# teasgen/speech_separation

Measured on AMD Instinct MI355X. Metric: mixtures/sec (2-spk, 4 s @ 8 kHz) DPTN-AV forward, higher is better.
Workload: dtype f32; 1 GPU; configs[2]: DPTN-AV (dptn_wav_av) forward, precomputed lip embeddings, batch=16 per GPU, T=32000, random-init weights (numpy seed 0); batch_per_gpu=16, samples=32000, parallelism=dp1 (batch shards, no data-path collective)

## Files before the change

speech_separation_amd/csrc/dptnav.hip:

```cpp
#include <hip/hip_runtime.h>

#include <cmath>
#include <cstdarg>
#include <cstdio>
#include <cstring>
#include <string>
#include <vector>

#include "../../include/dptnav.h"
#include "attention.h"
#include "attn_long_train.h"
#include "attn_block.h"
#include "attn_block64.h"
#include "common.h"
#include "gemm_ws.h"
#include "headtail.h"
#include "lstm.h"
#include "lstm16.h"
#include "fcln.h"
#include "dgrad_t.h"
#include "dgrad_r.h"
#include "gemm_t.h"
#include "sisnr.h"
#include "train_tail.h"
// ... 4 lines not shown
namespace {

thread_local std::string g_create_error;

struct PathWeights {
  const float *in_w, *in_b, *out_w, *out_b, *ln1_w, *ln1_b;
  const float *w_ih[2], *w_hh[2], *b_ih[2], *b_hh[2];
  const float *ffn_w, *ffn_b, *ln2_w, *ln2_b;
  int ndir;
};

constexpr int QUEUE_SLOTS = 1024;

struct Plan {
  int64_t L, S, M;
  size_t queue, vid, E, X0, X1, qkv, att, y1, pre, hc, stamps, wfold, wpack, wih, whh4, winp, wmask, total;
  size_t qkv_n, att_n, y1_n, hc_n;
};

struct Run {
  float* ws;
  Plan pl;
  hipStream_t st;
  int slot;
  hipEvent_t lstm_wait = nullptr;
  hipEvent_t lstm_record = nullptr;
  int half = 0;
  bool packed_whh4 = false;
  bool packed_inw = false;
  bool packed_wih = false;
  bool fuse128 = false;
  int batch_total = 0;
  bool packed = false;
  unsigned* take_queue(int n) {
    unsigned* q = reinterpret_cast<unsigned*>(ws + pl.queue) + slot;
    slot += n;
    return q;
  }
};

}

enum ProfCat { CAT_VIDEO = 0, CAT_ENCODER, CAT_QKV, CAT_ATTN, CAT_OUTPROJ, CAT_LSTM_PRE, CAT_LSTM, CAT_FFN,
// ... 4 lines not shown

struct ProfRec {
  int cat;
  hipEvent_t a, b;
};

struct dptnav_ctx {
  dptnav_config cfg;
  bool prof_on = false;
  bool opt_lstm_stamps = false;
  bool opt_overlap = true;
  bool opt_serialize = false;
  bool opt_lstm16 = true;
  int opt_fuse_pre128 = 1;
  int opt_lstm_sched = 1;
  bool fuse128_for(int B) const { return opt_fuse_pre128 == 2 || (opt_fuse_pre128 == 1 && B >= 12); }
  int opt_fcln = 1;
  bool opt_fuse_pre = true;
  bool opt_pack_whh = true;
  bool opt_pack_wih = true;
  bool opt_deterministic = false;
  int opt_lstm4 = 1;
  bool opt_split_bf16 = false;
  bool opt_fuse_attn = true;
  bool opt_gemm_t = true;
  bool opt_dgrad_r = true;
  bool opt_dgrad_t = true;
  bool opt_attn_v2 = true;
  int opt_attn_persist = 1;
  bool opt_fold_tail = true;
// ... 275 lines not shown
  p->X1 = take((size_t)p->M * N);
  p->qkv_n = (size_t)p->M * 3 * N;
  p->qkv = take(p->qkv_n);
  p->att_n = (size_t)p->M * N;
  p->att = take(std::max(p->att_n, (size_t)2 * B * p->L * 8));
  p->y1_n = (size_t)p->M * N;
  p->y1 = take(p->y1_n);
  p->pre = take((size_t)2 * pre_tiles * 512 * 32);
  p->hc_n = (size_t)p->M * 2 * H;
  p->hc = take(p->hc_n + (size_t)p->S * g.chunk_size * 2 * H);
  p->stamps = take((size_t)2 * 2 * (nst_a > nst_e ? nst_a : nst_e) * 4 * 4 * 2);
  p->wfold = take((size_t)8 * 2 * N + 8);
  p->wpack = take(g.arch == 0 && N == 128 ? (size_t)2 * g.num_blocks * ATTN_PACK_FLOATS : 0);
  p->wih = take((size_t)2 * g.num_blocks * 2 * 4 * H * N);
  p->whh4 = take((size_t)2 * g.num_blocks * 2 * 4 * H * H);
  p->winp = take(g.arch == 0 && N == 128 ? (size_t)2 * g.num_blocks * 3 * N * N : 0);
  p->wmask = take(g.mask_tail ? (size_t)2 * N * N + 2 * N : 0);
  p->total = o;
  return DPTNAV_OK;
}

#define LAUNCH_CHECK(c, what)                                                                  \
  do {                                                                                          \
    if ((c)->opt_debug_sync) fprintf(stderr, "[dptnav] launched %s\n", what);                   \
    hipError_t e_ = hipGetLastError();                                                          \
    if (e_ != hipSuccess) return (c)->fail(DPTNAV_ERR_HIP, "%s: %s", what, hipGetErrorString(e_)); \
  } while (0)

template <class Kern>
int set_lds(dptnav_ctx* c, Kern kern, size_t bytes, const char* what) {
// ... 419 lines not shown
    } else if (use16) {
      EpiLstmPre16 ep{pre, {w.b_ih[0], w.b_ih[1]}, {w.b_hh[0], w.b_hh[1]}, geom, nst16};
      rc = launch_gemm<N, 4, 1, 4>(c, run, CAT_LSTM_PRE, "lstm-pre gemm", wih0, nt4, w.ndir, al, ep, wih1, ldw_ih);
    } else if (split) {
      EpiLstmPre ep{pre, {w.b_ih[0], w.b_ih[1]}, {w.b_hh[0], w.b_hh[1]}, geom};
      rc = launch_gemm<N, 4, 1, 4, false, true>(c, run, CAT_LSTM_PRE, "lstm-pre gemm (split)", w.w_ih[0], nt4, w.ndir, al, ep, w.w_ih[1]);
    } else {
      EpiLstmPre ep{pre, {w.b_ih[0], w.b_ih[1]}, {w.b_hh[0], w.b_hh[1]}, geom};
      rc = launch_gemm<N, 4, 1, 4>(c, run, CAT_LSTM_PRE, "lstm-pre gemm", wih0, nt4, w.ndir, al, ep, wih1, ldw_ih);
    }
    if (rc) return rc;
  }
  if (run.lstm_wait && hipStreamWaitEvent(st, run.lstm_wait, 0) != hipSuccess)
    return c->fail(DPTNAV_ERR_HIP, "lstm stagger wait");
  if (usex) {
    ProfScope ps(c, CAT_LSTM, st);
    const int rc = lstm16x_launch(N, dptn, nst16, w.ndir, st, lstm_in, N, w.w_ih, w.b_ih, w.b_hh, w.w_hh, hc, w.ndir * LSTM_H,
                                  M, geom, c->opt_lstm_sched);
    if (rc != 0) return c->fail(DPTNAV_ERR_HIP, "lstm16x: %s", hipGetErrorString((hipError_t)rc));
  } else if (use16 && split) {
    ProfScope ps(c, CAT_LSTM, st);
    const int rc = lstm16s_launch(c->cfg.arch == 0, nst16, w.ndir, st, pre, w.w_hh[0], w.w_hh[1], hc, w.ndir * LSTM_H, (int)M, geom);
    if (rc != 0) return c->fail(DPTNAV_ERR_HIP, "lstm16s: %s", hipGetErrorString((hipError_t)rc));
  } else if (use4) {
    const float *whh0 = w.w_hh[0], *whh1 = w.w_hh[1];
    if (c->opt_pack_whh && 2 * (int)c->pw.size() <= LSTM4_PACK_MAX) {
      float* base = ws + pl.whh4;
      if (!run.packed_whh4) {
        const float* src[LSTM4_PACK_MAX];
        for (size_t i = 0; i < c->pw.size(); ++i) {
          src[2 * i] = c->pw[i].w_hh[0];
          src[2 * i + 1] = c->pw[i].ndir == 2 ? c->pw[i].w_hh[1] : nullptr;
        }
// ... 1060 lines not shown
  if (ws == nullptr || ((uintptr_t)ws & 255) != 0)
    return c->fail(DPTNAV_ERR_WORKSPACE, "workspace must be non-null and 256-byte aligned");
  if (ws_bytes < pl->total * sizeof(float))
    return c->fail(DPTNAV_ERR_WORKSPACE, "workspace too small: %zu < %zu bytes", ws_bytes, pl->total * sizeof(float));
  return DPTNAV_OK;
}

int begin_run(dptnav_ctx* c, Run* run, float* ws, const Plan& pl, hipStream_t st) {
  run->ws = ws;
  run->pl = pl;
  run->st = st;
  run->slot = 0;
  run->packed = false;
  run->packed_wih = false;
  run->packed_whh4 = false;
  hipError_t e = hipMemsetAsync(ws + pl.queue, 0, QUEUE_SLOTS * sizeof(unsigned), st);
  if (e != hipSuccess) return c->fail(DPTNAV_ERR_HIP, "ticket counter reset: %s", hipGetErrorString(e));
  return DPTNAV_OK;
}

int join_after(dptnav_ctx* c, hipStream_t st, bool forked, int rc_body, int nstreams = 2) {
  if (!forked) return rc_body;
  const std::string body_err = c->err;
  bool ok = true;
  for (int s = 0; s < nstreams; ++s)
    ok &= hipEventRecord(c->ev_join[s], c->streams[s]) == hipSuccess && hipStreamWaitEvent(st, c->ev_join[s], 0) == hipSuccess;
  if (rc_body) {
    c->err = body_err;
    return rc_body;
  }
// ... 713 lines not shown

int dptnav_set_option(dptnav_handle h, const char* key, int value) {
  if (!h || !key) return DPTNAV_ERR_INVALID;
  const std::string k(key);
  if (k == "lstm_stamps") h->opt_lstm_stamps = value != 0;
  else if (k == "dropout_ppm" && value >= 0 && value < 1000000) h->opt_dropout_ppm = value;
  else if (k == "dropout_seed") h->opt_dropout_seed = (unsigned)value;
  else if (k == "overlap") h->opt_overlap = value != 0;
  else if (k == "serialize") h->opt_serialize = value != 0;
  else if (k == "deterministic") h->opt_deterministic = value != 0;
  else if (k == "pack_wih") h->opt_pack_wih = value != 0;
  else if (k == "fuse_pre") h->opt_fuse_pre = value != 0;
  else if (k == "fcln" && value >= 0 && value <= 2) h->opt_fcln = value;
  else if (k == "fuse_pre128" && value >= 0 && value <= 2) h->opt_fuse_pre128 = value;
  else if (k == "lstm_sched" && value >= 0 && value <= 1) h->opt_lstm_sched = value;
  else if (k == "pack_whh") h->opt_pack_whh = value != 0;
  else if (k == "lstm16") h->opt_lstm16 = value != 0;
  else if (k == "lstm4") {
    if (value < 0 || value > 2) return h->fail(DPTNAV_ERR_INVALID, "lstm4: 0, 1 or 2");
    h->opt_lstm4 = (int)value;
  }
  else if (k == "fuse_attn") h->opt_fuse_attn = value != 0;
  else if (k == "attn_v2") h->opt_attn_v2 = value != 0;
  else if (k == "attn_persist" && value >= 0) h->opt_attn_persist = value;
  else if (k == "dgrad_t") h->opt_dgrad_t = value != 0;
  else if (k == "dgrad_r") h->opt_dgrad_r = value != 0;
  else if (k == "gemm_t") h->opt_gemm_t = value != 0;
  else if (k == "fuse_ffn") h->opt_fuse_ffn = value != 0;
  else if (k == "wgrad2") h->opt_wgrad2 = value != 0;
  else if (k == "ln_tape") h->opt_ln_tape = value != 0;
// ... 78 lines not shown
```

speech_separation_amd/csrc/lstm16.h:

```cpp
#pragma once
#include "common.h"

constexpr int L16_H = 128;
constexpr int L16_LDH = L16_H + 8;
constexpr int L16_HS_FLOATS = 2 * 16 * L16_LDH;
constexpr int L16_PRE_FLOATS = 4 * 8 * 256;
constexpr size_t L16_LDS_BYTES = sizeof(float) * (L16_HS_FLOATS + L16_PRE_FLOATS);
constexpr int L16_TILE_FLOATS = 4 * L16_H * 16;

DEV constexpr float l16_gate_scale(int gate) { return gate == 2 ? -2.8853900817779268f : -1.4426950408889634f; }

DEV int64_t pre16_tile_offset(int d, int st16, int t, int nst16, int len) {
  return (((int64_t)d * nst16 + st16) * len + t) * (int64_t)L16_TILE_FLOATS;
}

constexpr int L16_VARIANT_TRAIN = 7;
int lstm16_launch(int variant, bool relu, int nst16, int ndir, void* stream, const float* pre, const float* whh_f,
                  const float* whh_b, float* hc, int ldh, int dump_row, const SeqGeom& g, unsigned long long* stamps,
                  float* tape_gates = nullptr, float* tape_c = nullptr);

int lstm16s_launch(bool relu, int nst16, int ndir, void* stream, const float* pre, const float* whh_f, const float* whh_b,
                   float* hc, int ldh, int dump_row, const SeqGeom& g);
int lstm32s_launch(bool relu, int nst, int ndir, void* stream, const float* pre, const float* whh_f, const float* whh_b, float* hc,
                   int ldh, int dump_row, const SeqGeom& g);

int lstm4_launch(bool relu, int nst4, int nst16, int ndir, void* stream, const float* pre, const float* whh_f,
                 const float* whh_b, float* hc, int ldh, int dump_row, const SeqGeom& g, bool packed = false);
constexpr int LSTM4_PACK_MAX = 24;
int lstm4_pack_launch(void* stream, const float* const* src, int n, float* dst);

int lstm16x_launch(int nin, bool relu, int nst16, int ndir, void* stream, const float* x, int ldx, const float* const* wih,
                   const float* const* bih, const float* const* bhh, const float* const* whh, float* hc, int ldh,
                   int64_t dump_row, const SeqGeom& g, int sched = 1);
```

speech_separation_amd/csrc/lstm16x.hip:

```cpp
#include <hip/hip_runtime.h>

#include "lstm16.h"
#include "vmem_asm.h"

namespace {

template <int NIN>
struct X16 {
  static constexpr int MK = NIN / 16;
  static constexpr int LDX = NIN + 8;
  static constexpr int WL_FLOATS = 4 * MK * 8 * 256;
  static constexpr int XS_FLOATS = 2 * 16 * LDX;
  static constexpr int NXL = (16 * NIN / 4) / 256;
  static constexpr size_t LDS_BYTES = sizeof(float) * (WL_FLOATS + L16_HS_FLOATS + XS_FLOATS);
  static_assert((16 * NIN / 4) % 256 == 0 && NIN % 16 == 0, "input tile / threads");
  static_assert(LDS_BYTES <= 160 * 1024, "W_ih must fit the LDS beside the h and x tiles");
};

template <int NIN, bool RELU>
__global__ __launch_bounds__(256) void lstm16x_kernel(const float* __restrict__ x, int ldx, const float* __restrict__ wih_f,
                                                       const float* __restrict__ wih_b, const float* __restrict__ bih_f,
                                                       const float* __restrict__ bih_b, const float* __restrict__ bhh_f,
                                                       const float* __restrict__ bhh_b, const float* __restrict__ whh_f,
                                                       const float* __restrict__ whh_b, float* __restrict__ hc, int ldh,
                                                       int64_t dump_row, SeqGeom g) {
  using Sh = X16<NIN>;
  constexpr int MK = Sh::MK, LDX = Sh::LDX, NXL = Sh::NXL;
  extern __shared__ __attribute__((aligned(16))) float smem[];
  float* Wl = smem;
  float* Hs = smem + Sh::WL_FLOATS;
  float* Xs = Hs + L16_HS_FLOATS;
  const int tid = threadIdx.x;
  const int w = __builtin_amdgcn_readfirstlane(tid >> 6);
  const int lane = tid & 63, i16 = lane & 15, ks = lane >> 4;
  const int st = blockIdx.x, d = blockIdx.y;
  const float* whh = d ? whh_b : whh_f;
  const float* wih = d ? wih_b : wih_f;
  const float* bih = d ? bih_b : bih_f;
  const float* bhh = d ? bhh_b : bhh_f;

  float wf[8][32];
  float bsc[8];
  float* wl_wave = Wl + w * (MK * 8 * 256) + lane * 4;
#pragma unroll
  for (int b = 0; b < 8; ++b) {
    const int row = (b >> 1) * L16_H + 32 * w + 16 * (b & 1) + i16;
    const float gs = l16_gate_scale(b >> 1);
    const float* wrow = whh + (int64_t)row * L16_H + 4 * ks;
#pragma unroll
    for (int m = 0; m < 8; ++m) {
      const float4 v = *reinterpret_cast<const float4*>(wrow + 16 * m);
      wf[b][4 * m + 0] = v.x * gs;
      wf[b][4 * m + 1] = v.y * gs;
      wf[b][4 * m + 2] = v.z * gs;
      wf[b][4 * m + 3] = v.w * gs;
    }
    bsc[b] = (bih[row] + bhh[row]) * gs;
    const float* irow = wih + (int64_t)row * NIN + 4 * ks;
#pragma unroll
    for (int m = 0; m < MK; ++m) {
      const float4 v = *reinterpret_cast<const float4*>(irow + 16 * m);
      *reinterpret_cast<float4*>(wl_wave + (m * 8 + b) * 256) = make_float4(v.x * gs, v.y * gs, v.z * gs, v.w * gs);
    }
  }
#pragma unroll
  for (int b = 0; b < 8; ++b)
#pragma unroll
    for (int i = 0; i < 32; ++i) asm volatile("" : "+a"(wf[b][i]));

  const int t0 = d ? g.len - 1 : 0, tdir = d ? -1 : 1;
  const int tstride = seq_token_stride(g);
  const int srow = 4 * w + (lane >> 5), scol = 4 * (lane & 31);
  char* hp[2];
  const int64_t hstep = (int64_t)tdir * tstride * ldh * 4;
#pragma unroll
  for (int j = 0; j < 2; ++j) {
    const int q = st * 16 + srow + 2 * j;
    const int64_t tokb = q < g.nseq ? seq_token_base(g, q) : dump_row;
    hp[j] = reinterpret_cast<char*>(hc) + ((tokb + (int64_t)t0 * tstride) * ldh + d * L16_H + scol) * 4;
  }
  const char* xp[NXL];
  int xoff[NXL];
  const int64_t xstep = (int64_t)tdir * tstride * ldx * 4;
// ... 10 lines not shown
    const int64_t adv = (int64_t)(s < g.len ? s : g.len - 1) * xstep;
#pragma unroll
    for (int i = 0; i < NXL; ++i) xr[i] = *reinterpret_cast<const float4*>(xp[i] + adv);
  };
  auto stage_x = [&](int buf) {
#pragma unroll
    for (int i = 0; i < NXL; ++i) *reinterpret_cast<float4*>(Xs + buf * 16 * LDX + xoff[i]) = xr[i];
  };
  load_x(0);
  stage_x(0);
  load_x(1);
  stage_x(1);
  load_x(2);
  for (int i = tid; i < 16 * L16_LDH; i += 256) Hs[i] = 0.f;
  f32x4v cst[2] = {(f32x4v){0.f, 0.f, 0.f, 0.f}, (f32x4v){0.f, 0.f, 0.f, 0.f}};
  __syncthreads();

  f32x4v acc[8];
  auto input_part = [&](int buf) {
#pragma unroll
    for (int b = 0; b < 8; ++b) acc[b] = (f32x4v){bsc[b], bsc[b], bsc[b], bsc[b]};
    const float* xrow = Xs + buf * 16 * LDX + i16 * LDX + 4 * ks;
    float4 xa[MK];
#pragma unroll
    for (int m = 0; m < MK; ++m) xa[m] = *reinterpret_cast<const float4*>(xrow + 16 * m);
    float4 wcur[8];
#pragma unroll
    for (int b = 0; b < 8; ++b) wcur[b] = *reinterpret_cast<const float4*>(wl_wave + b * 256);
#pragma unroll
    for (int m = 0; m < MK; ++m) {
// ... 78 lines not shown
      if (hf == 0) cell_half(0);
    }
    cell_half(1);
    if (step + 1 < g.len) input_part((step + 1) & 1);
    __syncthreads();
  }
  {
    const float* hfin = Hs + (g.len & 1) * 16 * L16_LDH;
#pragma unroll
    for (int j = 0; j < 2; ++j) {
      float4 v = *reinterpret_cast<const float4*>(hfin + (srow + 2 * j) * L16_LDH + scol);
      if (RELU) v = make_float4(relu1(v.x), relu1(v.y), relu1(v.z), relu1(v.w));
      *reinterpret_cast<float4*>(hp[j]) = v;
    }
  }
}

constexpr int X128_RES = 33;
constexpr int X128_WL_FLOATS = 4 * (64 - X128_RES) * 256;
constexpr int X128_XS_FLOATS = 16 * 128;
constexpr size_t X128_LDS_BYTES = sizeof(float) * (X128_WL_FLOATS + L16_HS_FLOATS + 2 * X128_XS_FLOATS);
static_assert(X128_LDS_BYTES <= 160 * 1024, "LDS budget");

DEV LstmCell2 lstm_cell2_fc(f32x2 ai, f32x2 af, f32x2 ag, f32x2 ao, f32x2 c_prev) {
  LstmCell2 r;
  r.i = rcp_2(1.0f + exp2_2(ai));
  r.f = rcp_2(1.0f + exp2_2(af));
  r.g = 2.0f * rcp_2(1.0f + exp2_2(ag)) - 1.0f;
  r.o = rcp_2(1.0f + exp2_2(ao));
  const f32x2 ig = r.i * r.g;
  r.c = (f32x2){__builtin_fmaf(r.f.x, c_prev.x, ig.x), __builtin_fmaf(r.f.y, c_prev.y, ig.y)};
  const f32x2 th = 2.0f * rcp_2(1.0f + exp2_2(r.c * -2.8853900817779268f)) - 1.0f;
  r.h = r.o * th;
  return r;
}

template <bool RELU, int SCHED>
__global__ __launch_bounds__(256) void lstm16x128_kernel(const float* __restrict__ x, int ldx, const float* __restrict__ wih_f,
                                                          const float* __restrict__ wih_b, const float* __restrict__ bih_f,
                                                          const float* __restrict__ bih_b, const float* __restrict__ bhh_f,
                                                          const float* __restrict__ bhh_b, const float* __restrict__ whh_f,
                                                          const float* __restrict__ whh_b, float* __restrict__ hc, int ldh,
                                                          int64_t dump_row, SeqGeom g) {
  constexpr int NIN = 128, RES = X128_RES;
  extern __shared__ __attribute__((aligned(16))) float smem[];
  float* Wl = smem;
  float* Hs = smem + X128_WL_FLOATS;
  float* Xs = Hs + L16_HS_FLOATS;
  const int tid = threadIdx.x;
  const int w = __builtin_amdgcn_readfirstlane(tid >> 6);
  const int lane = tid & 63, i16 = lane & 15, ks = lane >> 4;
  const int st = blockIdx.x, d = blockIdx.y;
  const float* whh = d ? whh_b : whh_f;
  const float* wih = d ? wih_b : wih_f;
  const float* bih = d ? bih_b : bih_f;
  const float* bhh = d ? bhh_b : bhh_f;

  float wf[8][32];
  float bsc[8];
  float* wl_wave = Wl + w * ((64 - RES) * 256) + lane * 4;
#pragma unroll
  for (int b = 0; b < 8; ++b) {
    const int row = (b >> 1) * L16_H + 32 * w + 16 * (b & 1) + i16;
    const float gs = l16_gate_scale(b >> 1);
    const float* wrow = whh + (int64_t)row * L16_H + 4 * ks;
#pragma unroll
    for (int m = 0; m < 8; ++m) {
      const float4 v = *reinterpret_cast<const float4*>(wrow + 16 * m);
      wf[b][4 * m + 0] = v.x * gs;
      wf[b][4 * m + 1] = v.y * gs;
      wf[b][4 * m + 2] = v.z * gs;
      wf[b][4 * m + 3] = v.w * gs;
    }
    bsc[b] = (bih[row] + bhh[row]) * gs;
  }
#pragma unroll
  for (int b = 0; b < 8; ++b)
#pragma unroll
    for (int i = 0; i < 32; ++i) asm volatile("" : "+a"(wf[b][i]));
  float wiv[RES][4];
#pragma unroll
  for (int p = 0; p < 64; ++p) {
    const int m = p >> 3, b = p & 7;
    const int row = (b >> 1) * L16_H + 32 * w + 16 * (b & 1) + i16;
    const float gs = l16_gate_scale(b >> 1);
    const float4 v = *reinterpret_cast<const float4*>(wih + (int64_t)row * NIN + 16 * m + 4 * ks);
    if (p < RES) {
      constexpr int dummy = 0;
      (void)dummy;
      wiv[p % RES][0] = v.x * gs;
      wiv[p % RES][1] = v.y * gs;
      wiv[p % RES][2] = v.z * gs;
      wiv[p % RES][3] = v.w * gs;
    } else {
      *reinterpret_cast<float4*>(wl_wave + (p - RES) * 256) = make_float4(v.x * gs, v.y * gs, v.z * gs, v.w * gs);
    }
  }
#pragma unroll
  for (int p = 0; p < RES; ++p)
#pragma unroll
    for (int i = 0; i < 4; ++i) asm volatile("" : "+v"(wiv[p][i]));

  const int t0 = d ? g.len - 1 : 0, tdir = d ? -1 : 1;
  const int tstride = seq_token_stride(g);
  const int srow = 4 * w + (lane >> 5), scol = 4 * (lane & 31);
  unsigned hp[2];
  const unsigned hstep = (unsigned)(tdir * tstride * ldh * 4);
#pragma unroll
  for (int j = 0; j < 2; ++j) {
    const int q = st * 16 + srow + 2 * j;
    const int64_t tokb = q < g.nseq ? seq_token_base(g, q) : dump_row;
    hp[j] = (unsigned)(((tokb + (int64_t)t0 * tstride) * ldh + d * L16_H + scol) * 4);
  }
  char* const hcb = reinterpret_cast<char*>(hc);
  unsigned xp[2];
  const unsigned xstep = (unsigned)(tdir * tstride * ldx * 4);
#pragma unroll
  for (int i = 0; i < 2; ++i) {
    const int row = 2 * (2 * w + i) + (lane >> 5);
    const int q = st * 16 + row;
    const int64_t tokb = seq_token_base(g, q < g.nseq ? q : g.nseq - 1);
    xp[i] = (unsigned)(((tokb + (int64_t)t0 * tstride) * ldx + 4 * ((lane & 31) ^ (row & 15))) * 4);
  }
  const uint32_t xs_lds = lds_addr(Xs);
  auto dma_x = [&](int s, int buf, int i) {
    const unsigned adv = (unsigned)(s < g.len ? s : g.len - 1) * xstep;
    const uint32_t dst = xs_lds + (uint32_t)((buf * X128_XS_FLOATS + (2 * w + i) * 256) * 4);
    dma_part<false>(x, xp[i] + adv, dst);
  };
  dma_x(0, 0, 0); dma_x(0, 0, 1);
  dma_x(1, 1, 0); dma_x(1, 1, 1);
  for (int i = tid; i < 16 * L16_LDH; i += 256) Hs[i] = 0.f;
  f32x4v cst[2] = {(f32x4v){0.f, 0.f, 0.f, 0.f}, (f32x4v){0.f, 0.f, 0.f, 0.f}};
  asm volatile("s_waitcnt vmcnt(0)" ::: "memory");
  __syncthreads();

  f32x4v acc[8];
  const int xlane = i16 * 128 + 4 * (ks ^ (i16 & 3));
  const int xq = i16 >> 2;
  const uint32_t wl_lds = (uint32_t)(uintptr_t)(const __attribute__((address_space(3))) void*)wl_wave;
  f32x2 x0;
  auto input_chunk0 = [&](float t0v, float t1v, int tt0) {
    const float av[2] = {t0v, t1v};
#pragma unroll
    for (int half = 0; half < 2; ++half)
#pragma unroll
      for (int tt = 0; tt < 2; ++tt)
#pragma unroll
        for (int j = 0; j < 4; ++j) {
// ... 58 lines not shown
    for (int hf = 0; hf < 2; ++hf) {
#pragma unroll
      for (int r = 0; r < 4; r += 2) {
        const LstmCell2 u = lstm_cell2_fc((f32x2){acc[hf][r], acc[hf][r + 1]}, (f32x2){acc[2 + hf][r], acc[2 + hf][r + 1]},
                                       (f32x2){acc[4 + hf][r], acc[4 + hf][r + 1]}, (f32x2){acc[6 + hf][r], acc[6 + hf][r + 1]},
                                       (f32x2){cst[hf][r], cst[hf][r + 1]});
        cst[hf][r] = u.c.x;
        cst[hf][r + 1] = u.c.y;
        hnext[(4 * ks + r) * L16_LDH + 32 * w + 16 * hf + i16] = u.h.x;
        hnext[(4 * ks + r + 1) * L16_LDH + 32 * w + 16 * hf + i16] = u.h.y;
      }
    }
  };
  if constexpr (SCHED == 0) {
    input_part(0);
    __syncthreads();

    for (int step = 0; step < g.len; ++step) {
      const float* hcur = Hs + (step & 1) * 16 * L16_LDH;
      float* hnext = Hs + ((step + 1) & 1) * 16 * L16_LDH;
      const float* arow = hcur + i16 * L16_LDH + 4 * ks;
      float4 hs = *reinterpret_cast<const float4*>(hcur + srow * L16_LDH + scol);
      float4 a = *reinterpret_cast<const float4*>(arow);
#pragma unroll
      for (int b = 0; b < 8; ++b) asm volatile("" : "+v"(acc[b]));
      input_chunk0(x0.x, x0.y, 0);
      __builtin_amdgcn_sched_barrier(0);
      const unsigned adv = step > 0 ? hstep : 0u;

#pragma unroll
// ... 77 lines not shown
        else wait_lds<keep>(fa[ch & 1][0], fa[ch & 1][1]);
        __builtin_amdgcn_sched_barrier(0);
#pragma unroll
        for (int tt = 0; tt < 4; ++tt) {
          if constexpr (p0 < RES) acc[p0 & 7] = mfma16(xf[m][tt], wiv[p0 < RES ? p0 : 0][tt], acc[p0 & 7]);
          else acc[p0 & 7] = mfma16(xf[m][tt], fa[ch & 1][0][tt], acc[p0 & 7]);
          acc[(p0 + 1) & 7] = mfma16(xf[m][tt], fa[ch & 1][1][tt], acc[(p0 + 1) & 7]);
        }
      });
    };
    f32x4v xc0, xc1;
    request_x(std::integral_constant<int, 0>{}, 0, xc0);
    request_x(std::integral_constant<int, 1>{}, 0, xc1);
    wait_lds<0>(xc0, xc1);
    input_part1(0, xc0, xc1);
    __syncthreads();

    auto one_step = [&](int step, auto LAST) {
      constexpr bool last = decltype(LAST)::value;
      const uint32_t hcur = hs_lds + (uint32_t)((step & 1) * (16 * L16_LDH * 4));
      float* hnext = Hs + ((step + 1) & 1) * 16 * L16_LDH;
      f32x4v hsv[2], af[8];
      lds_read4_uncounted<0>(hsv[0], hcur + hrow_off);
      lds_read4_uncounted<2 * L16_LDH * 4>(hsv[1], hcur + hrow_off);
      lds_read4_uncounted<0>(af[0], hcur + a_off);
#pragma unroll
      for (int b = 0; b < 8; ++b) asm volatile("" : "+v"(acc[b]));
      input_chunk0(x0.x, x0.y, 0);
      const unsigned adv = step > 0 ? hstep : 0u;

// ... 40 lines not shown
    };
    for (int step = 0; step + 1 < g.len; ++step) one_step(step, std::false_type{});
    one_step(g.len - 1, std::true_type{});
  }
  {
    const float* hfin = Hs + (g.len & 1) * 16 * L16_LDH;
#pragma unroll
    for (int j = 0; j < 2; ++j) {
      float4 v = *reinterpret_cast<const float4*>(hfin + (srow + 2 * j) * L16_LDH + scol);
      if (RELU) v = make_float4(relu1(v.x), relu1(v.y), relu1(v.z), relu1(v.w));
      *reinterpret_cast<float4*>(hcb + hp[j]) = v;
    }
  }
}

}

int lstm16x_launch(int nin, bool relu, int nst16, int ndir, void* stream, const float* x, int ldx, const float* const* wih,
                   const float* const* bih, const float* const* bhh, const float* const* whh, float* hc, int ldh,
                   int64_t dump_row, const SeqGeom& g, int sched) {
  if ((nin != 64 && nin != 128) || nst16 < 1 || ndir < 1 || ndir > 2 || g.len < 1) return (int)hipErrorInvalidValue;
  auto kern = nin == 64 ? (relu ? lstm16x_kernel<64, true> : lstm16x_kernel<64, false>)
                        : sched == 0 ? (relu ? lstm16x128_kernel<true, 0> : lstm16x128_kernel<false, 0>)
                                     : (relu ? lstm16x128_kernel<true, 1> : lstm16x128_kernel<false, 1>);
  const size_t lds = nin == 64 ? X16<64>::LDS_BYTES : X128_LDS_BYTES;
  static PerDeviceOnce ready[6];
  const int dev = current_hip_device();
  const int ki = (nin == 128 ? (sched == 0 ? 4 : 2) : 0) + (relu ? 1 : 0);
  if (!ready[ki].done(dev)) {
    hipError_t e = hipFuncSetAttribute(reinterpret_cast<const void*>(kern), hipFuncAttributeMaxDynamicSharedMemorySize, (int)lds);
    if (e != hipSuccess) return (int)e;
    ready[ki].set(dev);
  }
  const int r = ndir == 2 ? 1 : 0;
  hipLaunchKernelGGL(kern, dim3(nst16, ndir), dim3(256), lds, static_cast<hipStream_t>(stream), x, ldx, wih[0], wih[r], bih[0],
                     bih[r], bhh[0], bhh[r], whh[0], whh[r], hc, ldh, dump_row, g);
  return (int)hipGetLastError();
}
```

speech_separation_amd/csrc/vmem_asm.h:

```cpp
#pragma once
#include "common.h"

DEV uint32_t lds_addr(const void* p) { return (uint32_t)(uintptr_t)(const __attribute__((address_space(3))) void*)p; }

template <bool HALF>
DEV void dma_part(const void* sbase, uint32_t voff, uint32_t lds_base) {
  if constexpr (!HALF) {
    asm volatile("s_mov_b32 m0, %0\n\ts_nop 4\n\tglobal_load_lds_dwordx4 %1, %2" ::"s"(lds_base), "v"(voff), "s"(sbase) : "memory", "m0");
  } else {
    uint32_t saved;
    asm volatile("s_mov_b32 m0, %1\n\ts_mov_b32 %0, exec_hi\n\ts_mov_b32 exec_hi, 0\n\ts_nop 4\n\tglobal_load_lds_dwordx4 %2, %3\n\ts_mov_b32 exec_hi, %0"
                 : "=&s"(saved)
                 : "s"(lds_base), "v"(voff), "s"(sbase)
                 : "memory", "m0");
  }
}
DEV void dma16(const void* g, uint32_t lds_base) {
  asm volatile("s_mov_b32 m0, %0\n\ts_nop 0\n\tglobal_load_lds_dwordx4 %1, off" ::"s"(lds_base), "v"(g) : "memory", "m0");
}

template <int OFF>
DEV void ldg4_uncounted(f32x4& dst, const void* sbase, uint32_t voff) {
  asm volatile("s_nop 4\n\tglobal_load_dwordx4 %0, %1, %2 offset:%3" : "=v"(dst) : "v"(voff), "s"(sbase), "n"(OFF) : "memory");
}
// ... 13 lines not shown
template <int KEEP>
DEV void wait_vm_v16(f32x4* r) {
  asm volatile("s_waitcnt vmcnt(%[n])"
               : "+v"(r[0]), "+v"(r[1]), "+v"(r[2]), "+v"(r[3]), "+v"(r[4]), "+v"(r[5]), "+v"(r[6]), "+v"(r[7]), "+v"(r[8]), "+v"(r[9]),
                 "+v"(r[10]), "+v"(r[11]), "+v"(r[12]), "+v"(r[13]), "+v"(r[14]), "+v"(r[15])
               : [n] "n"(KEEP)
               : "memory");
}
template <int KEEP>
DEV void wait_vm_a16(f32x4* r) {
  asm volatile("s_waitcnt vmcnt(%[n])"
               : "+a"(r[0]), "+a"(r[1]), "+a"(r[2]), "+a"(r[3]), "+a"(r[4]), "+a"(r[5]), "+a"(r[6]), "+a"(r[7]), "+a"(r[8]), "+a"(r[9]),
                 "+a"(r[10]), "+a"(r[11]), "+a"(r[12]), "+a"(r[13]), "+a"(r[14]), "+a"(r[15])
               : [n] "n"(KEEP)
               : "memory");
}
template <int KEEP>
DEV void wait_vm1(int& r) {
  asm volatile("s_waitcnt vmcnt(%[n])" : "+v"(r) : [n] "n"(KEEP) : "memory");
}
template <int KEEP>
DEV void retire_vm1(int r) {
  asm volatile("s_waitcnt vmcnt(%[n])" ::"v"(r), [n] "n"(KEEP) : "memory");
}

template <int OFF>
DEV void lds_read4_uncounted(f32x4v& dst, uint32_t addr) {
  asm volatile("ds_read_b128 %0, %1 offset:%2" : "=v"(dst) : "v"(addr), "n"(OFF) : "memory");
}
template <int KEEP>
// ... 77 lines not shown
```

Before: 582.4 mixtures/sec.

## Prepack LSTM16x weights once and stream them asynchronously in the kernel prologue

Adds a one-time pack kernel that pre-scales W_ih, W_hh and the fused biases into a per-wave, lane-contiguous layout in the workspace. The LSTM16x kernels then load weights from the packed buffer using uncounted vector loads and direct-to-LDS DMA. In the 128-input kernel, the W_hh register loads are deferred until after the first input step, so they overlap with setup work. This is meant to shorten the serial per-launch prologue, but it adds workspace, an extra pack launch per run, and more register and vmcnt bookkeeping.

```diff
diff --git a/speech_separation_amd/csrc/dptnav.hip b/speech_separation_amd/csrc/dptnav.hip
--- a/speech_separation_amd/csrc/dptnav.hip
+++ b/speech_separation_amd/csrc/dptnav.hip
@@ -42,7 +42,7 @@
 
 struct Plan {
   int64_t L, S, M;
-  size_t queue, vid, E, X0, X1, qkv, att, y1, pre, hc, stamps, wfold, wpack, wih, whh4, winp, wmask, total;
+  size_t queue, vid, E, X0, X1, qkv, att, y1, pre, hc, stamps, wfold, wpack, wih, whh4, x16pack, winp, wmask, total;
   size_t qkv_n, att_n, y1_n, hc_n;
 };
 
@@ -55,6 +55,7 @@
   hipEvent_t lstm_record = nullptr;
   int half = 0;
   bool packed_whh4 = false;
+  bool packed_x16 = false;
   bool packed_inw = false;
   bool packed_wih = false;
   bool fuse128 = false;
@@ -89,6 +90,7 @@
   bool opt_lstm16 = true;
   int opt_fuse_pre128 = 1;
   int opt_lstm_sched = 1;
+  int opt_lstm_prologue = 1;
   bool fuse128_for(int B) const { return opt_fuse_pre128 == 2 || (opt_fuse_pre128 == 1 && B >= 12); }
   int opt_fcln = 1;
   bool opt_fuse_pre = true;
@@ -394,6 +396,7 @@
   p->wpack = take(g.arch == 0 && N == 128 ? (size_t)2 * g.num_blocks * ATTN_PACK_FLOATS : 0);
   p->wih = take((size_t)2 * g.num_blocks * 2 * 4 * H * N);
   p->whh4 = take((size_t)2 * g.num_blocks * 2 * 4 * H * H);
+  p->x16pack = take((N == 64 || N == 128) && H == LSTM_H ? (size_t)2 * g.num_blocks * 2 * lstm16x_pack_floats((int)N) : 0);
   p->winp = take(g.arch == 0 && N == 128 ? (size_t)2 * g.num_blocks * 3 * N * N : 0);
   p->wmask = take(g.mask_tail ? (size_t)2 * N * N + 2 * N : 0);
   p->total = o;
@@ -843,9 +846,33 @@
   if (run.lstm_wait && hipStreamWaitEvent(st, run.lstm_wait, 0) != hipSuccess)
     return c->fail(DPTNAV_ERR_HIP, "lstm stagger wait");
   if (usex) {
+    const float* xpack = nullptr;
+    if (c->opt_lstm_prologue) {
+      float* base = ws + pl.x16pack;
+      if (!run.packed_x16) {
+        const int nmat = 2 * (int)c->pw.size();
+        for (int first = 0; first < nmat; first += LSTM16X_PACK_MAX) {
+          const float *s_ih[LSTM16X_PACK_MAX], *s_hh[LSTM16X_PACK_MAX], *s_bi[LSTM16X_PACK_MAX], *s_bh[LSTM16X_PACK_MAX];
+          const int n = std::min(LSTM16X_PACK_MAX, nmat - first);
+          for (int i = 0; i < n; ++i) {
+            const PathWeights& q = c->pw[(size_t)(first + i) / 2];
+            const int dir = (first + i) & 1;
+            const bool have = dir == 0 || q.ndir == 2;
+            s_ih[i] = have ? q.w_ih[dir] : nullptr;
+            s_hh[i] = have ? q.w_hh[dir] : nullptr;
+            s_bi[i] = have ? q.b_ih[dir] : nullptr;
+            s_bh[i] = have ? q.b_hh[dir] : nullptr;
+          }
+          const int rcp = lstm16x_pack_launch(N, st, s_ih, s_hh, s_bi, s_bh, n, base + (size_t)first * lstm16x_pack_floats(N));
+          if (rcp != 0) return c->fail(DPTNAV_ERR_HIP, "lstm16x weight pack: %s", hipGetErrorString((hipError_t)rcp));
+        }
+        run.packed_x16 = true;
+      }
+      xpack = base + (size_t)(2 * (2 * block + path)) * lstm16x_pack_floats(N);
+    }
     ProfScope ps(c, CAT_LSTM, st);
     const int rc = lstm16x_launch(N, dptn, nst16, w.ndir, st, lstm_in, N, w.w_ih, w.b_ih, w.b_hh, w.w_hh, hc, w.ndir * LSTM_H,
-                                  M, geom, c->opt_lstm_sched);
+                                  M, geom, c->opt_lstm_sched, xpack);
     if (rc != 0) return c->fail(DPTNAV_ERR_HIP, "lstm16x: %s", hipGetErrorString((hipError_t)rc));
   } else if (use16 && split) {
     ProfScope ps(c, CAT_LSTM, st);
@@ -1936,6 +1963,7 @@
   run->packed = false;
   run->packed_wih = false;
   run->packed_whh4 = false;
+  run->packed_x16 = false;
   hipError_t e = hipMemsetAsync(ws + pl.queue, 0, QUEUE_SLOTS * sizeof(unsigned), st);
   if (e != hipSuccess) return c->fail(DPTNAV_ERR_HIP, "ticket counter reset: %s", hipGetErrorString(e));
   return DPTNAV_OK;
@@ -2679,6 +2707,7 @@
   else if (k == "fcln" && value >= 0 && value <= 2) h->opt_fcln = value;
   else if (k == "fuse_pre128" && value >= 0 && value <= 2) h->opt_fuse_pre128 = value;
   else if (k == "lstm_sched" && value >= 0 && value <= 1) h->opt_lstm_sched = value;
+  else if (k == "lstm_prologue" && value >= 0 && value <= 1) h->opt_lstm_prologue = value;
   else if (k == "pack_whh") h->opt_pack_whh = value != 0;
   else if (k == "lstm16") h->opt_lstm16 = value != 0;
   else if (k == "lstm4") {
diff --git a/speech_separation_amd/csrc/lstm16.h b/speech_separation_amd/csrc/lstm16.h
--- a/speech_separation_amd/csrc/lstm16.h
+++ b/speech_separation_amd/csrc/lstm16.h
@@ -31,4 +31,8 @@
 
 int lstm16x_launch(int nin, bool relu, int nst16, int ndir, void* stream, const float* x, int ldx, const float* const* wih,
                    const float* const* bih, const float* const* bhh, const float* const* whh, float* hc, int ldh,
-                   int64_t dump_row, const SeqGeom& g, int sched = 1);
+                   int64_t dump_row, const SeqGeom& g, int sched = 1, const float* pack = nullptr);
+constexpr int LSTM16X_PACK_MAX = 24;
+constexpr size_t lstm16x_pack_floats(int nin) { return (size_t)4 * (8 * (nin / 16) + 66) * 256; }
+int lstm16x_pack_launch(int nin, void* stream, const float* const* wih, const float* const* whh, const float* const* bih,
+                        const float* const* bhh, int n, float* dst);
diff --git a/speech_separation_amd/csrc/lstm16x.hip b/speech_separation_amd/csrc/lstm16x.hip
--- a/speech_separation_amd/csrc/lstm16x.hip
+++ b/speech_separation_amd/csrc/lstm16x.hip
@@ -17,13 +17,20 @@
   static_assert(LDS_BYTES <= 160 * 1024, "W_ih must fit the LDS beside the h and x tiles");
 };
 
-template <int NIN, bool RELU>
-__global__ __launch_bounds__(256) void lstm16x_kernel(const float* __restrict__ x, int ldx, const float* __restrict__ wih_f,
-                                                       const float* __restrict__ wih_b, const float* __restrict__ bih_f,
-                                                       const float* __restrict__ bih_b, const float* __restrict__ bhh_f,
-                                                       const float* __restrict__ bhh_b, const float* __restrict__ whh_f,
-                                                       const float* __restrict__ whh_b, float* __restrict__ hc, int ldh,
-                                                       int64_t dump_row, SeqGeom g) {
+template <int NIN>
+struct XPack {
+  static constexpr int HH0 = 8 * (NIN / 16), BIAS0 = HH0 + 64, SETS = BIAS0 + 2;
+  static constexpr size_t DIR_FLOATS = (size_t)4 * SETS * 256;
+  static_assert(DIR_FLOATS == lstm16x_pack_floats(NIN), "lstm16.h");
+};
+
+template <int NIN, bool RELU, int PRO>
+DEV void lstm16x_body(const float* __restrict__ x, int ldx, const float* __restrict__ wih_f,
+                      const float* __restrict__ wih_b, const float* __restrict__ bih_f,
+                      const float* __restrict__ bih_b, const float* __restrict__ bhh_f,
+                      const float* __restrict__ bhh_b, const float* __restrict__ whh_f,
+                      const float* __restrict__ whh_b, const float* __restrict__ pk, float* __restrict__ hc, int ldh,
+                      int64_t dump_row, SeqGeom g) {
   using Sh = X16<NIN>;
   constexpr int MK = Sh::MK, LDX = Sh::LDX, NXL = Sh::NXL;
   extern __shared__ __attribute__((aligned(16))) float smem[];
@@ -42,31 +49,49 @@
   float wf[8][32];
   float bsc[8];
   float* wl_wave = Wl + w * (MK * 8 * 256) + lane * 4;
-#pragma unroll
-  for (int b = 0; b < 8; ++b) {
-    const int row = (b >> 1) * L16_H + 32 * w + 16 * (b & 1) + i16;
-    const float gs = l16_gate_scale(b >> 1);
-    const float* wrow = whh + (int64_t)row * L16_H + 4 * ks;
-#pragma unroll
-    for (int m = 0; m < 8; ++m) {
-      const float4 v = *reinterpret_cast<const float4*>(wrow + 16 * m);
-      wf[b][4 * m + 0] = v.x * gs;
-      wf[b][4 * m + 1] = v.y * gs;
-      wf[b][4 * m + 2] = v.z * gs;
-      wf[b][4 * m + 3] = v.w * gs;
-    }
-    bsc[b] = (bih[row] + bhh[row]) * gs;
-    const float* irow = wih + (int64_t)row * NIN + 4 * ks;
-#pragma unroll
-    for (int m = 0; m < MK; ++m) {
-      const float4 v = *reinterpret_cast<const float4*>(irow + 16 * m);
-      *reinterpret_cast<float4*>(wl_wave + (m * 8 + b) * 256) = make_float4(v.x * gs, v.y * gs, v.z * gs, v.w * gs);
-    }
-  }
-#pragma unroll
-  for (int b = 0; b < 8; ++b)
-#pragma unroll
-    for (int i = 0; i < 32; ++i) asm volatile("" : "+a"(wf[b][i]));
+  f32x4 wq[64], bq[2];
+  if constexpr (PRO == 0) {
+#pragma unroll
+    for (int b = 0; b < 8; ++b) {
+      const int row = (b >> 1) * L16_H + 32 * w + 16 * (b & 1) + i16;
+      const float gs = l16_gate_scale(b >> 1);
+      const float* wrow = whh + (int64_t)row * L16_H + 4 * ks;
+#pragma unroll
+      for (int m = 0; m < 8; ++m) {
+        const float4 v = *reinterpret_cast<const float4*>(wrow + 16 * m);
+        wf[b][4 * m + 0] = v.x * gs;
+        wf[b][4 * m + 1] = v.y * gs;
+        wf[b][4 * m + 2] = v.z * gs;
+        wf[b][4 * m + 3] = v.w * gs;
+      }
+      bsc[b] = (bih[row] + bhh[row]) * gs;
+      const float* irow = wih + (int64_t)row * NIN + 4 * ks;
+#pragma unroll
+      for (int m = 0; m < MK; ++m) {
+        const float4 v = *reinterpret_cast<const float4*>(irow + 16 * m);
+        *reinterpret_cast<float4*>(wl_wave + (m * 8 + b) * 256) = make_float4(v.x * gs, v.y * gs, v.z * gs, v.w * gs);
+      }
+    }
+#pragma unroll
+    for (int b = 0; b < 8; ++b)
+#pragma unroll
+      for (int i = 0; i < 32; ++i) asm volatile("" : "+a"(wf[b][i]));
+  } else {
+    using P = XPack<NIN>;
+    const char* pw = reinterpret_cast<const char*>(pk) + (size_t)(d * 4 + w) * (P::SETS * 1024);
+    const uint32_t lane16 = (uint32_t)lane * 16u;
+    const uint32_t wl_lds = lds_addr(Wl + w * (MK * 8 * 256));
+    static_for<8 * MK>([&](auto PP) {
+      constexpr int p = decltype(PP)::value;
+      dma_part<false>(pw + p * 1024, lane16, wl_lds + p * 1024);
+    });
+    ldg4_uncounted<0>(bq[0], pw + P::BIAS0 * 1024, lane16);
+    ldg4_uncounted<1024>(bq[1], pw + P::BIAS0 * 1024, lane16);
+    static_for<64>([&](auto Q) {
+      constexpr int q = decltype(Q)::value;
+      ldg4_uncounted_a<(q & 3) * 1024>(wq[q], pw + (P::HH0 + (q & ~3)) * 1024, lane16);
+    });
+  }
 
   const int t0 = d ? g.len - 1 : 0, tdir = d ? -1 : 1;
   const int tstride = seq_token_stride(g);
@@ -107,6 +132,20 @@
   load_x(2);
   for (int i = tid; i < 16 * L16_LDH; i += 256) Hs[i] = 0.f;
   f32x4v cst[2] = {(f32x4v){0.f, 0.f, 0.f, 0.f}, (f32x4v){0.f, 0.f, 0.f, 0.f}};
+  if constexpr (PRO == 1) {
+    static_for<4>([&](auto Q) { wait_vm_a16<0>(wq + 16 * decltype(Q)::value); });
+    wait_vm_v2<0>(bq[0], bq[1]);
+#pragma unroll
+    for (int b = 0; b < 8; ++b) {
+      bsc[b] = bq[b >> 2][b & 3];
+#pragma unroll
+      for (int i = 0; i < 32; ++i) wf[b][i] = wq[8 * b + (i >> 2)][i & 3];
+    }
+#pragma unroll
+    for (int b = 0; b < 8; ++b)
+#pragma unroll
+      for (int i = 0; i < 32; ++i) asm volatile("" : "+a"(wf[b][i]));
+  }
   __syncthreads();
 
   f32x4v acc[8];
@@ -215,6 +254,21 @@
       *reinterpret_cast<float4*>(hp[j]) = v;
     }
   }
+}
+
+#define LSTM16X_ARGS                                                                                                         \
+  const float *__restrict__ x, int ldx, const float *__restrict__ wih_f, const float *__restrict__ wih_b,                    \
+      const float *__restrict__ bih_f, const float *__restrict__ bih_b, const float *__restrict__ bhh_f,                     \
+      const float *__restrict__ bhh_b, const float *__restrict__ whh_f, const float *__restrict__ whh_b,                     \
+      const float *__restrict__ pk, float *__restrict__ hc, int ldh, int64_t dump_row, SeqGeom g
+#define LSTM16X_PASS x, ldx, wih_f, wih_b, bih_f, bih_b, bhh_f, bhh_b, whh_f, whh_b, pk, hc, ldh, dump_row, g
+template <int NIN, bool RELU>
+__global__ __launch_bounds__(256) void lstm16x_kernel(LSTM16X_ARGS) {
+  lstm16x_body<NIN, RELU, 1>(LSTM16X_PASS);
+}
+template <int NIN, bool RELU>
+__global__ __launch_bounds__(256) void lstm16x_pro0_kernel(LSTM16X_ARGS) {
+  lstm16x_body<NIN, RELU, 0>(LSTM16X_PASS);
 }
 
 constexpr int X128_RES = 33;
@@ -236,13 +290,8 @@
   return r;
 }
 
-template <bool RELU, int SCHED>
-__global__ __launch_bounds__(256) void lstm16x128_kernel(const float* __restrict__ x, int ldx, const float* __restrict__ wih_f,
-                                                          const float* __restrict__ wih_b, const float* __restrict__ bih_f,
-                                                          const float* __restrict__ bih_b, const float* __restrict__ bhh_f,
-                                                          const float* __restrict__ bhh_b, const float* __restrict__ whh_f,
-                                                          const float* __restrict__ whh_b, float* __restrict__ hc, int ldh,
-                                                          int64_t dump_row, SeqGeom g) {
+template <bool RELU, int SCHED, int PRO>
+DEV void lstm16x128_body(LSTM16X_ARGS) {
   constexpr int NIN = 128, RES = X128_RES;
   extern __shared__ __attribute__((aligned(16))) float smem[];
   float* Wl = smem;
@@ -260,47 +309,49 @@
   float wf[8][32];
   float bsc[8];
   float* wl_wave = Wl + w * ((64 - RES) * 256) + lane * 4;
-#pragma unroll
-  for (int b = 0; b < 8; ++b) {
-    const int row = (b >> 1) * L16_H + 32 * w + 16 * (b & 1) + i16;
-    const float gs = l16_gate_scale(b >> 1);
-    const float* wrow = whh + (int64_t)row * L16_H + 4 * ks;
-#pragma unroll
-    for (int m = 0; m < 8; ++m) {
-      const float4 v = *reinterpret_cast<const float4*>(wrow + 16 * m);
-      wf[b][4 * m + 0] = v.x * gs;
-      wf[b][4 * m + 1] = v.y * gs;
-      wf[b][4 * m + 2] = v.z * gs;
-      wf[b][4 * m + 3] = v.w * gs;
-    }
-    bsc[b] = (bih[row] + bhh[row]) * gs;
-  }
-#pragma unroll
-  for (int b = 0; b < 8; ++b)
-#pragma unroll
-    for (int i = 0; i < 32; ++i) asm volatile("" : "+a"(wf[b][i]));
   float wiv[RES][4];
-#pragma unroll
-  for (int p = 0; p < 64; ++p) {
-    const int m = p >> 3, b = p & 7;
-    const int row = (b >> 1) * L16_H + 32 * w + 16 * (b & 1) + i16;
-    const float gs = l16_gate_scale(b >> 1);
-    const float4 v = *reinterpret_cast<const float4*>(wih + (int64_t)row * NIN + 16 * m + 4 * ks);
-    if (p < RES) {
-      constexpr int dummy = 0;
-      (void)dummy;
-      wiv[p % RES][0] = v.x * gs;
-      wiv[p % RES][1] = v.y * gs;
-      wiv[p % RES][2] = v.z * gs;
-      wiv[p % RES][3] = v.w * gs;
-    } else {
-      *reinterpret_cast<float4*>(wl_wave + (p - RES) * 256) = make_float4(v.x * gs, v.y * gs, v.z * gs, v.w * gs);
-    }
-  }
-#pragma unroll
-  for (int p = 0; p < RES; ++p)
-#pragma unroll
-    for (int i = 0; i < 4; ++i) asm volatile("" : "+v"(wiv[p][i]));
+  if constexpr (PRO == 0) {
+#pragma unroll
+    for (int b = 0; b < 8; ++b) {
+      const int row = (b >> 1) * L16_H + 32 * w + 16 * (b & 1) + i16;
+      const float gs = l16_gate_scale(b >> 1);
+      const float* wrow = whh + (int64_t)row * L16_H + 4 * ks;
+#pragma unroll
+      for (int m = 0; m < 8; ++m) {
+        const float4 v = *reinterpret_cast<const float4*>(wrow + 16 * m);
+        wf[b][4 * m + 0] = v.x * gs;
+        wf[b][4 * m + 1] = v.y * gs;
+        wf[b][4 * m + 2] = v.z * gs;
+        wf[b][4 * m + 3] = v.w * gs;
+      }
+      bsc[b] = (bih[row] + bhh[row]) * gs;
+    }
+#pragma unroll
+    for (int b = 0; b < 8; ++b)
+#pragma unroll
+      for (int i = 0; i < 32; ++i) asm volatile("" : "+a"(wf[b][i]));
+#pragma unroll
+    for (int p = 0; p < 64; ++p) {
+      const int m = p >> 3, b = p & 7;
+      const int row = (b >> 1) * L16_H + 32 * w + 16 * (b & 1) + i16;
+      const float gs = l16_gate_scale(b >> 1);
+      const float4 v = *reinterpret_cast<const float4*>(wih + (int64_t)row * NIN + 16 * m + 4 * ks);
+      if (p < RES) {
+        constexpr int dummy = 0;
+        (void)dummy;
+        wiv[p % RES][0] = v.x * gs;
+        wiv[p % RES][1] = v.y * gs;
+        wiv[p % RES][2] = v.z * gs;
+        wiv[p % RES][3] = v.w * gs;
+      } else {
+        *reinterpret_cast<float4*>(wl_wave + (p - RES) * 256) = make_float4(v.x * gs, v.y * gs, v.z * gs, v.w * gs);
+      }
+    }
+#pragma unroll
+    for (int p = 0; p < RES; ++p)
+#pragma unroll
+      for (int i = 0; i < 4; ++i) asm volatile("" : "+v"(wiv[p][i]));
+  }
 
   const int t0 = d ? g.len - 1 : 0, tdir = d ? -1 : 1;
   const int tstride = seq_token_stride(g);
@@ -331,9 +382,61 @@
   };
   dma_x(0, 0, 0); dma_x(0, 0, 1);
   dma_x(1, 1, 0); dma_x(1, 1, 1);
+  f32x4 wq[64], wiq[RES], bq[2];
+  auto request_whh = [&](auto Q) {
+    constexpr int q = decltype(Q)::value;
+    const char* pw = reinterpret_cast<const char*>(pk) + (size_t)(d * 4 + w) * (XPack<128>::SETS * 1024);
+    ldg4_uncounted_a<(q & 3) * 1024>(wq[q], pw + (XPack<128>::HH0 + (q & ~3)) * 1024, (uint32_t)lane * 16u);
+  };
+  auto whh_landed = [&]() {
+    if constexpr (PRO == 1) {
+      static_for<4>([&](auto Q) { wait_vm_a16<0>(wq + 16 * decltype(Q)::value); });
+#pragma unroll
+      for (int b = 0; b < 8; ++b)
+#pragma unroll
+        for (int i = 0; i < 32; ++i) wf[b][i] = wq[8 * b + (i >> 2)][i & 3];
+      if constexpr (SCHED == 0) {
+#pragma unroll
+        for (int b = 0; b < 8; ++b)
+#pragma unroll
+          for (int i = 0; i < 32; ++i) asm volatile("" : "+a"(wf[b][i]));
+      }
+    }
+  };
+  if constexpr (PRO == 1) {
+    using P = XPack<128>;
+    const char* pw = reinterpret_cast<const char*>(pk) + (size_t)(d * 4 + w) * (P::SETS * 1024);
+    const uint32_t lane16 = (uint32_t)lane * 16u;
+    const uint32_t wl_dma = lds_addr(Wl + w * ((64 - RES) * 256));
+    ldg4_uncounted<0>(bq[0], pw + P::BIAS0 * 1024, lane16);
+    ldg4_uncounted<1024>(bq[1], pw + P::BIAS0 * 1024, lane16);
+    static_for<64>([&](auto PP) {
+      constexpr int p = decltype(PP)::value;
+      if constexpr (p < RES) ldg4_uncounted<(p & 3) * 1024>(wiq[p < RES ? p : 0], pw + (p & ~3) * 1024, lane16);
+      else dma_part<false>(pw + p * 1024, lane16, wl_dma + (p - RES) * 1024);
+    });
+    static_for<60>(request_whh);
+  }
   for (int i = tid; i < 16 * L16_LDH; i += 256) Hs[i] = 0.f;
   f32x4v cst[2] = {(f32x4v){0.f, 0.f, 0.f, 0.f}, (f32x4v){0.f, 0.f, 0.f, 0.f}};
-  asm volatile("s_waitcnt vmcnt(0)" ::: "memory");
+  if constexpr (PRO == 0) {
+    asm volatile("s_waitcnt vmcnt(0)" ::: "memory");
+  } else {
+    wait_vm_v16<60>(wiq);
+    wait_vm_v16<60>(wiq + 16);
+    wait_vm_v3<60>(wiq[32], bq[0], bq[1]);
+    static_assert(RES == 33, "the three waits above name every resident set");
+    request_whh(std::integral_constant<int, 60>{});
+    request_whh(std::integral_constant<int, 61>{});
+    request_whh(std::integral_constant<int, 62>{});
+    request_whh(std::integral_constant<int, 63>{});
+#pragma unroll
+    for (int b = 0; b < 8; ++b) bsc[b] = bq[b >> 2][b & 3];
+#pragma unroll
+    for (int p = 0; p < RES; ++p)
+#pragma unroll
+      for (int i = 0; i < 4; ++i) wiv[p][i] = wiq[p][i];
+  }
   __syncthreads();
 
   f32x4v acc[8];
@@ -422,6 +525,7 @@
   };
   if constexpr (SCHED == 0) {
     input_part(0);
+    whh_landed();
     __syncthreads();
 
     for (int step = 0; step < g.len; ++step) {
@@ -529,6 +633,7 @@
     request_x(std::integral_constant<int, 1>{}, 0, xc1);
     wait_lds<0>(xc0, xc1);
     input_part1(0, xc0, xc1);
+    whh_landed();
     __syncthreads();
 
     auto one_step = [&](int step, auto LAST) {
@@ -599,19 +704,82 @@
   }
 }
 
+template <bool RELU, int SCHED>
+__global__ __launch_bounds__(256) void lstm16x128_kernel(LSTM16X_ARGS) {
+  lstm16x128_body<RELU, SCHED, 1>(LSTM16X_PASS);
+}
+template <bool RELU, int SCHED>
+__global__ __launch_bounds__(256) void lstm16x128_pro0_kernel(LSTM16X_ARGS) {
+  lstm16x128_body<RELU, SCHED, 0>(LSTM16X_PASS);
+}
+
+struct Lstm16xPackArgs {
+  const float *wih[LSTM16X_PACK_MAX], *whh[LSTM16X_PACK_MAX], *bih[LSTM16X_PACK_MAX], *bhh[LSTM16X_PACK_MAX];
+};
+template <int NIN>
+__global__ __launch_bounds__(256) void lstm16x_pack_kernel(Lstm16xPackArgs a, float* __restrict__ dst) {
+  using P = XPack<NIN>;
+  const float *wih = a.wih[blockIdx.y], *whh = a.whh[blockIdx.y], *bih = a.bih[blockIdx.y], *bhh = a.bhh[blockIdx.y];
+  if (wih == nullptr) return;
+  float4* out = reinterpret_cast<float4*>(dst + (size_t)blockIdx.y * P::DIR_FLOATS);
+  for (int f = blockIdx.x * 256 + threadIdx.x; f < 4 * P::SETS * 64; f += gridDim.x * 256) {
+    const int lane = f & 63, set = (f >> 6) % P::SETS, w = (f >> 6) / P::SETS;
+    const int i16 = lane & 15, ks = lane >> 4;
+    float4 v;
+    if (set < P::BIAS0) {
+      const bool hh = set >= P::HH0;
+      const int b = hh ? (set - P::HH0) >> 3 : set & 7, m = hh ? (set - P::HH0) & 7 : set >> 3;
+      const int row = (b >> 1) * L16_H + 32 * w + 16 * (b & 1) + i16;
+      const float gs = l16_gate_scale(b >> 1);
+      const float* src = hh ? whh + (size_t)row * L16_H + 16 * m + 4 * ks : wih + (size_t)row * NIN + 16 * m + 4 * ks;
+      const float4 s = *reinterpret_cast<const float4*>(src);
+      v = make_float4(s.x * gs, s.y * gs, s.z * gs, s.w * gs);
+    } else {
+      float r[4];
+#pragma unroll
+      for (int k = 0; k < 4; ++k) {
+        const int b = 4 * (set - P::BIAS0) + k;
+        const int row = (b >> 1) * L16_H + 32 * w + 16 * (b & 1) + i16;
+        r[k] = (bih[row] + bhh[row]) * l16_gate_scale(b >> 1);
+      }
+      v = make_float4(r[0], r[1], r[2], r[3]);
+    }
+    out[f] = v;
+  }
+}
+
+}
+
+int lstm16x_pack_launch(int nin, void* stream, const float* const* wih, const float* const* whh, const float* const* bih,
+                        const float* const* bhh, int n, float* dst) {
+  if ((nin != 64 && nin != 128) || n < 1 || n > LSTM16X_PACK_MAX || dst == nullptr) return (int)hipErrorInvalidValue;
+  Lstm16xPackArgs a;
+  for (int i = 0; i < LSTM16X_PACK_MAX; ++i) {
+    a.wih[i] = i < n ? wih[i] : nullptr;
+    a.whh[i] = i < n ? whh[i] : nullptr;
+    a.bih[i] = i < n ? bih[i] : nullptr;
+    a.bhh[i] = i < n ? bhh[i] : nullptr;
+  }
+  if (nin == 64) hipLaunchKernelGGL(lstm16x_pack_kernel<64>, dim3(16, n), dim3(256), 0, static_cast<hipStream_t>(stream), a, dst);
+  else hipLaunchKernelGGL(lstm16x_pack_kernel<128>, dim3(16, n), dim3(256), 0, static_cast<hipStream_t>(stream), a, dst);
+  return (int)hipGetLastError();
 }
 
 int lstm16x_launch(int nin, bool relu, int nst16, int ndir, void* stream, const float* x, int ldx, const float* const* wih,
                    const float* const* bih, const float* const* bhh, const float* const* whh, float* hc, int ldh,
-                   int64_t dump_row, const SeqGeom& g, int sched) {
+                   int64_t dump_row, const SeqGeom& g, int sched, const float* pack) {
   if ((nin != 64 && nin != 128) || nst16 < 1 || ndir < 1 || ndir > 2 || g.len < 1) return (int)hipErrorInvalidValue;
-  auto kern = nin == 64 ? (relu ? lstm16x_kernel<64, true> : lstm16x_kernel<64, false>)
-                        : sched == 0 ? (relu ? lstm16x128_kernel<true, 0> : lstm16x128_kernel<false, 0>)
-                                     : (relu ? lstm16x128_kernel<true, 1> : lstm16x128_kernel<false, 1>);
+  const bool pro = pack != nullptr;
+  auto kern = nin == 64 ? (pro ? (relu ? lstm16x_kernel<64, true> : lstm16x_kernel<64, false>)
+                               : (relu ? lstm16x_pro0_kernel<64, true> : lstm16x_pro0_kernel<64, false>))
+              : pro    ? (sched == 0 ? (relu ? lstm16x128_kernel<true, 0> : lstm16x128_kernel<false, 0>)
+                                     : (relu ? lstm16x128_kernel<true, 1> : lstm16x128_kernel<false, 1>))
+                       : (sched == 0 ? (relu ? lstm16x128_pro0_kernel<true, 0> : lstm16x128_pro0_kernel<false, 0>)
+                                     : (relu ? lstm16x128_pro0_kernel<true, 1> : lstm16x128_pro0_kernel<false, 1>));
   const size_t lds = nin == 64 ? X16<64>::LDS_BYTES : X128_LDS_BYTES;
-  static PerDeviceOnce ready[6];
+  static PerDeviceOnce ready[12];
   const int dev = current_hip_device();
-  const int ki = (nin == 128 ? (sched == 0 ? 4 : 2) : 0) + (relu ? 1 : 0);
+  const int ki = 2 * ((nin == 128 ? (sched == 0 ? 4 : 2) : 0) + (relu ? 1 : 0)) + (pro ? 1 : 0);
   if (!ready[ki].done(dev)) {
     hipError_t e = hipFuncSetAttribute(reinterpret_cast<const void*>(kern), hipFuncAttributeMaxDynamicSharedMemorySize, (int)lds);
     if (e != hipSuccess) return (int)e;
@@ -619,6 +787,6 @@
   }
   const int r = ndir == 2 ? 1 : 0;
   hipLaunchKernelGGL(kern, dim3(nst16, ndir), dim3(256), lds, static_cast<hipStream_t>(stream), x, ldx, wih[0], wih[r], bih[0],
-                     bih[r], bhh[0], bhh[r], whh[0], whh[r], hc, ldh, dump_row, g);
+                     bih[r], bhh[0], bhh[r], whh[0], whh[r], pack, hc, ldh, dump_row, g);
   return (int)hipGetLastError();
 }
diff --git a/speech_separation_amd/csrc/vmem_asm.h b/speech_separation_amd/csrc/vmem_asm.h
--- a/speech_separation_amd/csrc/vmem_asm.h
+++ b/speech_separation_amd/csrc/vmem_asm.h
@@ -51,6 +51,14 @@
                  "+a"(r[10]), "+a"(r[11]), "+a"(r[12]), "+a"(r[13]), "+a"(r[14]), "+a"(r[15])
                : [n] "n"(KEEP)
                : "memory");
+}
+template <int KEEP>
+DEV void wait_vm_v2(f32x4& r0, f32x4& r1) {
+  asm volatile("s_waitcnt vmcnt(%[n])" : "+v"(r0), "+v"(r1) : [n] "n"(KEEP) : "memory");
+}
+template <int KEEP>
+DEV void wait_vm_v3(f32x4& r0, f32x4& r1, f32x4& r2) {
+  asm volatile("s_waitcnt vmcnt(%[n])" : "+v"(r0), "+v"(r1), "+v"(r2) : [n] "n"(KEEP) : "memory");
 }
 template <int KEEP>
 DEV void wait_vm1(int& r) {
```

Measured after the change: 589.9 mixtures/sec, median of 6. 1.01x the previous value.
